# CPJKU/beat_this

Measured on NVIDIA H100. Metric: clips/sec (30 s audio->beats, final0), higher is better.
Workload: dtype f16

## Files before the change

beat_this_b200/csrc/kernels_attn.cu:

```cuda
#include <cstdio>

#include "tc_common.cuh"

namespace bt {

constexpr int AT_BQ = 128;
constexpr int AT_BKV = 64;
constexpr int AT_NST = 4;
constexpr int AT_WARPS = 8;
constexpr int AT_THREADS = 32 * (AT_WARPS + 1);
constexpr int AT_SQ = AT_BQ * 64;
constexpr int AT_SKV = AT_BKV * 64;
constexpr int AT_SMEM = 1024 + AT_SQ + AT_NST * 2 * AT_SKV + 128;

constexpr uint32_t AT_POLY_MASK = 0x52u;

__device__ __forceinline__ uint32_t sw64_off(int r, int c) {
  return static_cast<uint32_t>(r * 64 + ((c ^ ((r >> 1) & 3)) << 4));
}

__global__ void __launch_bounds__(AT_THREADS, 2)
attn_time_kernel(const __grid_constant__ CUtensorMap tmQ, const __grid_constant__ CUtensorMap tmKV,
                 const float* __restrict__ gates, h16* __restrict__ out, int L, int heads,
                 const ChunkSrc* __restrict__ chunks, int seqs_per_chunk) {
  extern __shared__ uint8_t smem_raw[];
  const uint32_t sbase = (smem_u32(smem_raw) + 1023u) & ~1023u;
  const uint32_t sQ = sbase;
  const uint32_t sK = sQ + AT_SQ;
  const uint32_t sV = sK + AT_NST * AT_SKV;
  const uint32_t bar_q = sV + AT_NST * AT_SKV;
  const uint32_t full = bar_q + 8;
  const uint32_t empty = full + 8 * AT_NST;

  const int warp = threadIdx.x >> 5, lane = threadIdx.x & 31;
  const int q0 = blockIdx.x * AT_BQ;
  const int h = blockIdx.y;
  const int seq = blockIdx.z;
  const int C = heads * 32;
  const int Lk = chunks ? chunks[seq / seqs_per_chunk].len : L;
  const int nkv = ceil_div(Lk, AT_BKV);

  if (threadIdx.x == 0) {
    mbar_init(bar_q, 1);
    for (int i = 0; i < AT_NST; ++i) {
      mbar_init(full + 8 * i, 1);
      mbar_init(empty + 8 * i, AT_WARPS);
    }
    fence_barrier_init();
  }
  __syncthreads();

  if (warp == AT_WARPS) {
    if (lane == 0) {
      tma_prefetch_desc(&tmQ);
      tma_prefetch_desc(&tmKV);
      mbar_expect_tx(bar_q, AT_SQ);
      tma_load_3d(sQ, &tmQ, bar_q, h * 32, q0, seq);
      for (int j = 0; j < nkv; ++j) {
        const int st = j % AT_NST;
        if (j >= AT_NST) mbar_wait(empty + 8 * st, ((j / AT_NST) - 1) & 1);
        mbar_expect_tx(full + 8 * st, 2 * AT_SKV);
        tma_load_3d(sK + st * AT_SKV, &tmKV, full + 8 * st, C + h * 32, j * AT_BKV, seq);
        tma_load_3d(sV + st * AT_SKV, &tmKV, full + 8 * st, 2 * C + h * 32, j * AT_BKV, seq);
      }
    }
    return;
  }

  const int r0 = warp * 16;
  mbar_wait(bar_q, 0);
  uint32_t qa[2][4];
#pragma unroll
  for (int ks = 0; ks < 2; ++ks) ldmatrix_x4(sQ + sw64_off(r0 + (lane & 15), 2 * ks + (lane >> 4)), qa[ks]);

  float o[4][4];
#pragma unroll
  for (int d = 0; d < 4; ++d) o[d][0] = o[d][1] = o[d][2] = o[d][3] = 0.f;
  float m_run[2] = {-INFINITY, -INFINITY}, l_run[2] = {0.f, 0.f};
  for (int j = 0; j < nkv; ++j) {
    const int st = j % AT_NST;
    mbar_wait(full + 8 * st, (j / AT_NST) & 1);
    const uint32_t kb = sK + st * AT_SKV, vb = sV + st * AT_SKV;
    float s[8][4];
#pragma unroll
    for (int nb = 0; nb < 8; ++nb) {
      s[nb][0] = s[nb][1] = s[nb][2] = s[nb][3] = 0.f;
      uint32_t kf[4];
      ldmatrix_x4(kb + sw64_off(nb * 8 + (lane & 7), lane >> 3), kf);
      mma_16816(s[nb], qa[0], kf[0], kf[1]);
      mma_16816(s[nb], qa[1], kf[2], kf[3]);
    }
    if (j == nkv - 1) {
      const int lim = Lk - j * AT_BKV;
#pragma unroll
      for (int nb = 0; nb < 8; ++nb) {
        const int key = nb * 8 + 2 * (lane & 3);
        if (key >= lim) s[nb][0] = s[nb][2] = -INFINITY;
        if (key + 1 >= lim) s[nb][1] = s[nb][3] = -INFINITY;
      }
    }
    float mx[2] = {-INFINITY, -INFINITY};
#pragma unroll
    for (int nb = 0; nb < 8; ++nb) {
      mx[0] = fmaxf(mx[0], fmaxf(s[nb][0], s[nb][1]));
      mx[1] = fmaxf(mx[1], fmaxf(s[nb][2], s[nb][3]));
    }
    float mref[2], alpha[2];
#pragma unroll
    for (int r = 0; r < 2; ++r) {
      mx[r] = fmaxf(mx[r], __shfl_xor_sync(0xffffffffu, mx[r], 1));
      mx[r] = fmaxf(mx[r], __shfl_xor_sync(0xffffffffu, mx[r], 2));
      mref[r] = fmaxf(m_run[r], mx[r]);
      alpha[r] = ex2_approx(m_run[r] - mref[r]);
      m_run[r] = mref[r];
      l_run[r] *= alpha[r];
    }
#pragma unroll
    for (int d = 0; d < 4; ++d) {
      o[d][0] *= alpha[0]; o[d][1] *= alpha[0];
      o[d][2] *= alpha[1]; o[d][3] *= alpha[1];
    }
    uint32_t pa[4][4];
#pragma unroll
    for (int nb = 0; nb < 8; ++nb) {
      float p[4];
#pragma unroll
      for (int i = 0; i < 4; ++i) {
        const float x = s[nb][i] - mref[i >> 1];
        p[i] = ((AT_POLY_MASK >> nb) & 1u) ? ex2_poly(x) : ex2_approx(x);
      }
      l_run[0] += p[0] + p[1];
      l_run[1] += p[2] + p[3];
      pa[nb >> 1][(nb & 1) * 2] = pack_h16x2(p[0], p[1]);
      pa[nb >> 1][(nb & 1) * 2 + 1] = pack_h16x2(p[2], p[3]);
    }
#pragma unroll
    for (int kk = 0; kk < 4; ++kk) {
      const int key = kk * 16 + (lane & 7) + ((lane >> 3) & 1) * 8;
#pragma unroll
      for (int dp = 0; dp < 2; ++dp) {
        uint32_t vf[4];
        ldmatrix_x4_trans(vb + sw64_off(key, 2 * dp + (lane >> 4)), vf);
        mma_16816(o[2 * dp], pa[kk], vf[0], vf[1]);
        mma_16816(o[2 * dp + 1], pa[kk], vf[2], vf[3]);
      }
    }
    __syncwarp();
    if (lane == 0) mbar_arrive(empty + 8 * st);
  }
#pragma unroll
  for (int r = 0; r < 2; ++r) {
    l_run[r] += __shfl_xor_sync(0xffffffffu, l_run[r], 1);
    l_run[r] += __shfl_xor_sync(0xffffffffu, l_run[r], 2);
  }
#pragma unroll
  for (int r = 0; r < 2; ++r) {
    const int q = q0 + r0 + (lane >> 2) + 8 * r;
    if (q < L) {
      const int64_t m = static_cast<int64_t>(seq) * L + q;
      const float gsc = gates[m * heads + h] / l_run[r];
      h16* dst = out + m * C + h * 32 + 2 * (lane & 3);
#pragma unroll
      for (int d = 0; d < 4; ++d)
        *reinterpret_cast<uint32_t*>(dst + 8 * d) = pack_h16x2(o[d][2 * r] * gsc, o[d][2 * r + 1] * gsc);
    }
  }
}

struct TcAttnPlan {
  CUtensorMap tmQ;
  CUtensorMap tmKV;
  int seqs, L, heads;
};

TcAttnPlan* tc_attn_plan_create(const void* qkv, int seqs, int L, int heads, char* err, int errlen) {
  TcAttnPlan* p = new TcAttnPlan();
  p->seqs = seqs; p->L = L; p->heads = heads;
  const int C = heads * 32;
  const uint64_t dims[3] = {static_cast<uint64_t>(3 * C), static_cast<uint64_t>(L), static_cast<uint64_t>(seqs)};
  const uint64_t strides[2] = {static_cast<uint64_t>(3 * C) * 2, static_cast<uint64_t>(L) * 3 * C * 2};
  const uint32_t box_q[3] = {32, AT_BQ, 1};
  const uint32_t box_kv[3] = {32, AT_BKV, 1};
  if (!make_tmap(&p->tmQ, qkv, 3, dims, strides, box_q, 64, err, errlen) ||
      !make_tmap(&p->tmKV, qkv, 3, dims, strides, box_kv, 64, err, errlen)) {
    delete p;
    return nullptr;
  }
  return p;
}
void tc_attn_plan_destroy(TcAttnPlan* p) { delete p; }

void launch_attn_time_tc(const TcAttnPlan* p, const float* gates, void* out, cudaStream_t st, const ChunkSrc* chunks,
                         int seqs_per_chunk) {
  dim3 grid(ceil_div(p->L, AT_BQ), p->heads, p->seqs);
  attn_time_kernel<<<grid, AT_THREADS, AT_SMEM, st>>>(p->tmQ, p->tmKV, gates, reinterpret_cast<h16*>(out), p->L, p->heads,
                                                      chunks, seqs_per_chunk);
}

int tc_init_attn(char* err, int errlen) {
  const cudaError_t r = cudaFuncSetAttribute(attn_time_kernel, cudaFuncAttributeMaxDynamicSharedMemorySize, AT_SMEM);
  if (r != cudaSuccess) {
    snprintf(err, errlen, "cudaFuncSetAttribute(attn_time_kernel) failed: %s", cudaGetErrorString(r));
    return -1;
  }
  return 0;
}

}
```

Measured before the change: 587.2.

## Drop dedicated producer warp and issue KV TMA loads from consumer thread

Removes the separate TMA producer warp so thread 0 of the first compute warp initially loads Q and the first NST KV stages, then refills each freed stage after all warps release it. This cuts the block from nine to eight warps and should lower register and scheduling overhead. The cost is that warp 0 blocks on the empty barrier until the slowest warp finishes each stage, which can stall that warp and serialize the pipeline. Swizzled ldmatrix offsets for K and V are also hoisted out of the loop as per-lane constants plus fixed strides.

```diff
diff --git a/beat_this_b200/csrc/kernels_attn.cu b/beat_this_b200/csrc/kernels_attn.cu
--- a/beat_this_b200/csrc/kernels_attn.cu
+++ b/beat_this_b200/csrc/kernels_attn.cu
@@ -8,7 +8,7 @@
 constexpr int AT_BKV = 64;
 constexpr int AT_NST = 4;
 constexpr int AT_WARPS = 8;
-constexpr int AT_THREADS = 32 * (AT_WARPS + 1);
+constexpr int AT_THREADS = 32 * AT_WARPS;
 constexpr int AT_SQ = AT_BQ * 64;
 constexpr int AT_SKV = AT_BKV * 64;
 constexpr int AT_SMEM = 1024 + AT_SQ + AT_NST * 2 * AT_SKV + 128;
@@ -40,7 +40,14 @@
   const int Lk = chunks ? chunks[seq / seqs_per_chunk].len : L;
   const int nkv = ceil_div(Lk, AT_BKV);
 
-  if (threadIdx.x == 0) {
+  auto load_kv = [&](int t) {
+    const int st = t % AT_NST;
+    mbar_expect_tx(full + 8 * st, 2 * AT_SKV);
+    tma_load_3d(sK + st * AT_SKV, &tmKV, full + 8 * st, C + h * 32, t * AT_BKV, seq);
+    tma_load_3d(sV + st * AT_SKV, &tmKV, full + 8 * st, 2 * C + h * 32, t * AT_BKV, seq);
+  };
+  const bool loader = threadIdx.x == 0;
+  if (loader) {
     mbar_init(bar_q, 1);
     for (int i = 0; i < AT_NST; ++i) {
       mbar_init(full + 8 * i, 1);
@@ -49,25 +56,18 @@
     fence_barrier_init();
   }
   __syncthreads();
-
-  if (warp == AT_WARPS) {
-    if (lane == 0) {
-      tma_prefetch_desc(&tmQ);
-      tma_prefetch_desc(&tmKV);
-      mbar_expect_tx(bar_q, AT_SQ);
-      tma_load_3d(sQ, &tmQ, bar_q, h * 32, q0, seq);
-      for (int j = 0; j < nkv; ++j) {
-        const int st = j % AT_NST;
-        if (j >= AT_NST) mbar_wait(empty + 8 * st, ((j / AT_NST) - 1) & 1);
-        mbar_expect_tx(full + 8 * st, 2 * AT_SKV);
-        tma_load_3d(sK + st * AT_SKV, &tmKV, full + 8 * st, C + h * 32, j * AT_BKV, seq);
-        tma_load_3d(sV + st * AT_SKV, &tmKV, full + 8 * st, 2 * C + h * 32, j * AT_BKV, seq);
-      }
-    }
-    return;
+  if (loader) {
+    tma_prefetch_desc(&tmQ);
+    tma_prefetch_desc(&tmKV);
+    mbar_expect_tx(bar_q, AT_SQ);
+    tma_load_3d(sQ, &tmQ, bar_q, h * 32, q0, seq);
+    for (int t = 0; t < nkv && t < AT_NST; ++t) load_kv(t);
   }
 
   const int r0 = warp * 16;
+  const uint32_t k_off = sw64_off(lane & 7, lane >> 3);
+  const int v_row = (lane & 7) + ((lane >> 3) & 1) * 8;
+  const uint32_t v_off[2] = {sw64_off(v_row, lane >> 4), sw64_off(v_row, 2 + (lane >> 4))};
   mbar_wait(bar_q, 0);
   uint32_t qa[2][4];
 #pragma unroll
@@ -86,7 +86,7 @@
     for (int nb = 0; nb < 8; ++nb) {
       s[nb][0] = s[nb][1] = s[nb][2] = s[nb][3] = 0.f;
       uint32_t kf[4];
-      ldmatrix_x4(kb + sw64_off(nb * 8 + (lane & 7), lane >> 3), kf);
+      ldmatrix_x4(kb + k_off + nb * 512, kf);
       mma_16816(s[nb], qa[0], kf[0], kf[1]);
       mma_16816(s[nb], qa[1], kf[2], kf[3]);
     }
@@ -136,17 +136,21 @@
     }
 #pragma unroll
     for (int kk = 0; kk < 4; ++kk) {
-      const int key = kk * 16 + (lane & 7) + ((lane >> 3) & 1) * 8;
 #pragma unroll
       for (int dp = 0; dp < 2; ++dp) {
         uint32_t vf[4];
-        ldmatrix_x4_trans(vb + sw64_off(key, 2 * dp + (lane >> 4)), vf);
+        ldmatrix_x4_trans(vb + v_off[dp] + kk * 1024, vf);
         mma_16816(o[2 * dp], pa[kk], vf[0], vf[1]);
         mma_16816(o[2 * dp + 1], pa[kk], vf[2], vf[3]);
       }
     }
     __syncwarp();
     if (lane == 0) mbar_arrive(empty + 8 * st);
+    if (loader && j + AT_NST < nkv) {
+      mbar_wait(empty + 8 * st, (j / AT_NST) & 1);
+      load_kv(j + AT_NST);
+    }
+    __syncwarp();
   }
 #pragma unroll
   for (int r = 0; r < 2; ++r) {
```

New measurement: 597.9, median of 6. 1.8% higher.
